# rubenwiersma/deltaconv

Measured on AMD Instinct MI355X. Metric: point-clouds/sec fwd+bwd, ModelNet40 1024pt k=20, 1/2/4/8 MI355X, higher is better.
Workload: dtype f32; 1 GPU; ModelNet40 classification, 1024 points, k=20, batch=32 per GPU, fwd+bwd+SGD step, train-mode BN/Dropout, HIP-graph replay; global_batch=32, parallelism=dp1

## Files before the change

deltaconv_amd/csrc/common.h:

```cpp
#pragma once
#include <hip/hip_runtime.h>
#include <stdint.h>
#include <stdio.h>

#define DC_EXPORT extern "C" __attribute__((visibility("default")))

enum {
    DC_OK = 0,
    DC_ERR_ARG = -1,
    DC_ERR_LAUNCH = -2,
    DC_ERR_WORKSPACE = -3
};

void dc_set_error(const char* fmt, ...);

#define DC_REQUIRE(cond, ...)                 \
    do {                                      \
        if (!(cond)) {                        \
            dc_set_error(__VA_ARGS__);        \
            return DC_ERR_ARG;                \
        }                                     \
    } while (0)

bool dc_ensure_lds(unsigned long long* done_mask, const void* kernel, size_t bytes, const char* what);
bool dc_take_lds_failure();

#define DC_CHECK_LAUNCH(name)                                                   \
    do {                                                                        \
        if (dc_take_lds_failure()) {                                            \
            (void)hipGetLastError();                                            \
            return DC_ERR_LAUNCH;                                               \
        }                                                                       \
        hipError_t e_ = hipGetLastError();                                      \
        if (e_ != hipSuccess) {                                                 \
            dc_set_error("%s: %s", name, hipGetErrorString(e_));                \
            return DC_ERR_LAUNCH;                                               \
        }                                                                       \
    } while (0)

enum { DC_OPT_XCD_REMAP = 0, DC_OPT_GATHER_BATCH = 1, DC_OPT_TN_LDS = 2 , DC_OPT_GEMM_EXACT = 3 , DC_OPT_GEMM_STAGGER = 4 , DC_OPT_TN_TILE = 5 , DC_OPT_TN_SLABS = 6 , DC_OPT_TILE_UPW = 7, DC_OPT_CSC_ONE_WG = 8 , DC_OPT_NO_PLANES = 9 , DC_OPT_CE_TWO_LAUNCH = 10 , DC_OPT_WIDE_TILES = 11 , DC_OPT_COUNT = 12 };
int dc_option(int key);

static inline int dc_cdiv(long long a, long long b) { return (int)((a + b - 1) / b); }

enum { DC_ST_TILE = 1 , DC_ST_ELL = 2 ,
       DC_ST_NN = 4 , DC_ST_GEMM = 8  };
#ifndef DC_NT_MASK
#define DC_NT_MASK (DC_ST_TILE)
#endif
typedef float dc_f32x4 __attribute__((ext_vector_type(4)));
template <int FAMILY>
__device__ __forceinline__ void dc_store16(float* p, dc_f32x4 v) {
    if constexpr ((DC_NT_MASK & FAMILY) != 0) __builtin_nontemporal_store(v, reinterpret_cast<dc_f32x4*>(p));
    else *reinterpret_cast<dc_f32x4*>(p) = v;
}

constexpr int DC_FIN_MAX = 4, DC_FIN_BLOB = 128;
enum { DC_FIN_BN = 0, DC_FIN_BWD_COEF = 1 };
struct DcFinPending {
    int kind, chunks, C;
    const double* partial;
    alignas(8) unsigned char blob[DC_FIN_BLOB];
    int stage1, rpc;
    long R;
    alignas(8) unsigned char functor[DC_FIN_BLOB];
};
bool dc_gemm_take_request();
void dc_gemm_flush(void* stream);
void dc_gemm_discard();
bool dc_fin_take_request();
void dc_fin_push(int kind, const double* partial, int chunks, int C, const void* fin, size_t bytes, const void* functor = nullptr,
                 size_t functor_bytes = 0, long R = 0, int rpc = 0);
int dc_fin_pending(DcFinPending** out);
// ... 46 lines not shown
```

deltaconv_amd/csrc/error.hip:

```cpp
#include <cstring>
#include "common.h"
#include <stdarg.h>

static thread_local char g_err[512] = "";

void dc_set_error(const char* fmt, ...) {
    va_list ap;
    va_start(ap, fmt);
    vsnprintf(g_err, sizeof(g_err), fmt, ap);
    va_end(ap);
}

DC_EXPORT const char* dc_last_error(void) { return g_err; }
DC_EXPORT int32_t dc_version(void) { return 100; }

static int g_opt[DC_OPT_COUNT] = {1};
int dc_option(int key) { return (key >= 0 && key < DC_OPT_COUNT) ? g_opt[key] : 0; }
DC_EXPORT int dc_set_option(int32_t key, int32_t value) {
    if (key < 0 || key >= DC_OPT_COUNT) return DC_ERR_ARG;
    g_opt[key] = value;
    return DC_OK;
}

static thread_local bool g_lds_failed = false;
bool dc_take_lds_failure() {
    const bool f = g_lds_failed;
    g_lds_failed = false;
    return f;
}
bool dc_ensure_lds(unsigned long long* done_mask, const void* kernel, size_t bytes, const char* what) {
    int dev = 0;
    if (hipGetDevice(&dev) != hipSuccess) dev = 0;
    const unsigned long long bit = dev < 64 ? 1ull << dev : 0ull;
    if (bit && (__atomic_load_n(done_mask, __ATOMIC_ACQUIRE) & bit)) return true;
    const hipError_t e = hipFuncSetAttribute(kernel, hipFuncAttributeMaxDynamicSharedMemorySize, (int)bytes);
    if (e != hipSuccess) {
        (void)hipGetLastError();
        dc_set_error("%s: needs %zu KiB of LDS per workgroup (MI355X / gfx950 offers 160 KiB); device %d refused: %s", what,
                     bytes / 1024, dev, hipGetErrorString(e));
        g_lds_failed = true;
        return false;
    }
    if (bit) __atomic_fetch_or(done_mask, bit, __ATOMIC_RELEASE);
    return true;
}

static thread_local DcFinPending g_fin[DC_FIN_MAX];
static thread_local int g_fin_count = 0;
static thread_local bool g_fin_open = false, g_fin_request = false, g_gemm_request = false;
bool dc_gemm_take_request() {
    const bool take = g_fin_open && g_gemm_request && g_fin_request;
    g_gemm_request = false;
    return take;
}
bool dc_fin_take_request() {
    const bool take = g_fin_open && g_fin_request && g_fin_count < DC_FIN_MAX;
    g_fin_request = false;
    return take;
}
void dc_fin_push(int kind, const double* partial, int chunks, int C, const void* fin, size_t bytes, const void* functor,
                 size_t functor_bytes, long R, int rpc) {
    DcFinPending& e = g_fin[g_fin_count++];
    e.kind = kind; e.partial = partial; e.chunks = chunks; e.C = C;
    memcpy(e.blob, fin, bytes);
    e.stage1 = functor != nullptr; e.R = R; e.rpc = rpc;
    if (functor) memcpy(e.functor, functor, functor_bytes);
}
int dc_fin_pending(DcFinPending** out) { *out = g_fin; return g_fin_count; }
void dc_fin_clear() { g_fin_count = 0; g_fin_open = false; g_fin_request = false; g_gemm_request = false; }
DC_EXPORT int dc_finalisers_begin(void) {
    if (g_fin_open) {
        dc_set_error("dc_finalisers_begin: a batch is already open on this thread");
        return DC_ERR_ARG;
    }
    g_fin_open = true; g_fin_count = 0; g_fin_request = false;
    return DC_OK;
}
DC_EXPORT int dc_finaliser_defer_next(void) {
    g_fin_request = g_fin_open;
    return DC_OK;
}
DC_EXPORT int dc_gemm_defer_next(void) {
    g_gemm_request = g_fin_open;
    return DC_OK;
// ... 23 lines not shown
```

deltaconv_amd/csrc/gemm.hip:

```cpp
#include <algorithm>
#include <type_traits>
#include "common.h"
#include "nn_math.h"
#include "colreduce.h"

namespace {

typedef float f32x16 __attribute__((ext_vector_type(16)));
typedef float f32x4 __attribute__((ext_vector_type(4)));

#ifndef DC_X3_PLAIN
#define DC_X3_PLAIN 2
#endif
#ifndef DC_X3_PRO
#define DC_X3_PRO 1
#endif
#ifdef DC_LAB_STAMPS
__device__ unsigned long long dc_lab_stamps[8192 * 8];
#define DC_STAMP(n) do { if (threadIdx.x == 0 && blockIdx.y == 0 && blockIdx.x < 8192) dc_lab_stamps[blockIdx.x * 8 + (n)] = __builtin_amdgcn_s_memtime(); } while (0)
#else
#define DC_STAMP(n) do { } while (0)
#endif
constexpr int BK = 32;
constexpr int LDK = BK + 4;
constexpr int NT = 256;

enum { EPI_NONE = 0, EPI_COLSTATS = 1, EPI_VNSTATS = 2 , EPI_VNSTATS0 = 3  };
enum { B_NK = 0 , B_KN = 1  };
enum { A_MK = 0 , A_KM = 1  };

struct GemmP {
    const float* A; long lda;
    const float* B; long ldb;
    float* C; long ldc;
    long M; int N; long K;
    int tiles_n, remap, accumulate;
    long k_per_slab, slab_stride;
    const float* A2; long lda2;
    const float* pc; int pcn;
    float slope;
    double* part; int chunks, stat_cols;
    int stagger, resident;
    const unsigned short* Bp; long bps;
};

typedef unsigned u32x4 __attribute__((ext_vector_type(4)));
__device__ __forceinline__ f32x4 uload4(const float* ubase, unsigned voff, unsigned soff = 0) {
    const __amdgpu_buffer_rsrc_t r = __builtin_amdgcn_make_buffer_rsrc(const_cast<float*>(ubase), 0, 0x7FFFFFFF, 0x00020000);
    const u32x4 v = __builtin_amdgcn_raw_buffer_load_b128(r, (int)voff, (int)soff, 0);
    return __builtin_bit_cast(f32x4, v);
}

constexpr unsigned POISON = 0x80000000u;
__device__ __forceinline__ f32x4 gload4v(const float* ubase, unsigned voff, unsigned soff, bool ok) {
    return uload4(ubase, ok ? voff : POISON, soff);
}
__device__ __forceinline__ f32x4 gload4s(const float* ubase, unsigned voff, unsigned soff, bool ok_row, long col, long ncols) {
    const __amdgpu_buffer_rsrc_t r = __builtin_amdgcn_make_buffer_rsrc(const_cast<float*>(ubase), 0, 0x7FFFFFFF, 0x00020000);
    f32x4 v;
#pragma unroll
    for (int e = 0; e < 4; ++e)
        v[e] = __builtin_bit_cast(float, __builtin_amdgcn_raw_buffer_load_b32(
                   r, (int)((ok_row && col + e < ncols) ? voff + 4u * e : POISON), (int)soff, 0));
    return v;
}
template <int MODE>
__device__ __forceinline__ f32x4 pload4(const float* ubase, unsigned voff, unsigned soff, bool ok_row, long col, long ncols) {
    if (MODE == 0) return uload4(ubase, voff, soff);
    if (MODE == 1) return gload4v(ubase, voff, soff, ok_row && col < ncols);
    return gload4s(ubase, voff, soff, ok_row, col, ncols);
}

__device__ __forceinline__ f32x4 bn_bwd_vec(const f32x4 dy, const f32x4 h, const f32x4 (&cf)[5], float slope) {
    f32x4 o;
#pragma unroll
    for (int e = 0; e < 4; ++e) {
        const float z = fmaf(cf[0][e], h[e], cf[1][e]);
        const float dz = dy[e] * (z > 0.f ? 1.f : slope);
        o[e] = fmaf(cf[2][e], dz, fmaf(cf[3][e], h[e], cf[4][e]));
// ... 2 lines not shown
}

__device__ __forceinline__ void lds_barrier() {
    __builtin_amdgcn_sched_barrier(0);
    asm volatile("s_waitcnt lgkmcnt(0)\n\ts_barrier" ::: "memory");
    __builtin_amdgcn_sched_barrier(0);
}

typedef __bf16 bf16x8 __attribute__((ext_vector_type(8)));
typedef __bf16 bf16x2 __attribute__((ext_vector_type(2)));
typedef float f32x2 __attribute__((ext_vector_type(2)));
struct Planes { u32x4 h, m, l; };
__device__ __forceinline__ unsigned pk_bf16(float a, float b) {
    return __builtin_bit_cast(unsigned, __builtin_convertvector((f32x2){a, b}, bf16x2));
}
__device__ __forceinline__ void split_pair(float x0, float x1, unsigned& h, unsigned& m, unsigned& l) {
    h = pk_bf16(x0, x1);
    const float r0 = x0 - __builtin_bit_cast(float, h << 16), r1 = x1 - __builtin_bit_cast(float, h & 0xFFFF0000u);
    m = pk_bf16(r0, r1);
    const float s0 = r0 - __builtin_bit_cast(float, m << 16), s1 = r1 - __builtin_bit_cast(float, m & 0xFFFF0000u);
    l = pk_bf16(s0, s1);
}
__device__ __forceinline__ void split8(const f32x4 a, const f32x4 b, Planes& o) {
    const float x[8] = {a[0], a[1], a[2], a[3], b[0], b[1], b[2], b[3]};
#pragma unroll
    for (int j = 0; j < 4; ++j) {
        unsigned h, m, l;
        split_pair(x[2 * j], x[2 * j + 1], h, m, l);
        o.h[j] = h; o.m[j] = m; o.l[j] = l;
    }
}
__device__ __forceinline__ f32x16 mfma_bf16(const u32x4 a, const u32x4 b, const f32x16 c) {
    return __builtin_amdgcn_mfma_f32_32x32x16_bf16(__builtin_bit_cast(bf16x8, a), __builtin_bit_cast(bf16x8, b), c, 0, 0, 0);
}

template <int BM, int BN, int AL, int BL, int MODE, int EPI, int PRO = 0, int X3 = 0, int BP = 0>
__device__ __forceinline__ void gemm_body(const GemmP& p, const unsigned bid, const unsigned gemm_blocks) {
    static_assert(!BP || (X3 == 2 && AL == A_MK && BL == B_NK && MODE == 0), "pre-split B planes: pipelined split loop, K-contiguous operands, whole tiles");
    constexpr bool FAST = MODE == 0;
    constexpr int MA = MODE == 0 ? 0 : (MODE == 1 || MODE == 3 ? 1 : 2), MB = MODE == 0 ? 0 : (MODE == 1 || MODE == 4 ? 1 : 2);
    constexpr int WM = BM / 2, WN = BN / 2;
    constexpr int TM = WM / 32, TN = WN / 32;
    constexpr int A_FL = AL == A_MK ? BM * LDK : BK * BM;
    constexpr int B_FL = BL == B_NK ? BN * LDK : BK * BN;
    constexpr int A_IT = BM / 32, B_IT = BP ? 0 : BN / 32;
    extern __shared__ __attribute__((aligned(16))) float smem[];
    float* As = smem;
    float* Bs = smem + 2 * A_FL;

    const int tid = threadIdx.x, lane = tid & 63, wave = tid >> 6;
    const int li = lane & 31, lh = lane >> 5;
    DC_STAMP(0);
    if (p.stagger > 0 && (long)blockIdx.y * gemm_blocks + bid < p.resident) {
        const unsigned slot = __builtin_amdgcn_s_getreg((3 << 11) | 4);
        if (slot & 1) {
            const unsigned long long t0 = __builtin_amdgcn_s_memtime();
            while (__builtin_amdgcn_s_memtime() - t0 < (unsigned long long)p.stagger) __builtin_amdgcn_s_sleep(16);
        }
    }
    long blk = bid;
    if (p.remap) {
        const long q = gemm_blocks >> 3, r = gemm_blocks & 7, xcd = blk & 7, idx = blk >> 3;
        blk = xcd * q + (xcd < r ? xcd : r) + idx;
    }
    const long kbeg = (long)blockIdx.y * p.k_per_slab;
    const long kend = min(p.K, kbeg + p.k_per_slab);
    const long tm = blk / p.tiles_n;
    const int tn = (int)(blk - tm * p.tiles_n);
    const long m0 = tm * BM;
    const int n0 = tn * BN;
    const int wm0 = (wave >> 1) * WM, wn0 = (wave & 1) * WN;

    f32x16 acc[TM][TN];
#pragma unroll
    for (int i = 0; i < TM; ++i)
#pragma unroll
        for (int j = 0; j < TN; ++j)
#pragma unroll
            for (int q = 0; q < 16; ++q) acc[i][j][q] = 0.f;

    constexpr int STG = (X3 || PRO || (BM == 128 && BN == 128 && BL == B_KN)) ? 1 : 2;
    f32x4 sa[STG][A_IT], sb[STG][B_IT ? B_IT : 1];
    f32x4 sa2[PRO ? A_IT : 1], cf[5];
    if (PRO && AL == A_KM) {
#pragma unroll
        for (int q = 0; q < 5; ++q)
            cf[q] = pload4<MODE == 0 ? 0 : 2>(p.pc + (long)q * p.pcn + m0, (unsigned)((tid % (BM / 4)) * 16), 0, true,
                                              m0 + (tid % (BM / 4)) * 4, p.M);
    }
    const unsigned voa = AL == A_MK ? (unsigned)(((tid >> 3) * p.lda + (tid & 7) * 4) * 4)
                                    : (unsigned)(((tid / (BM / 4)) * p.lda + (tid % (BM / 4)) * 4) * 4);
    const unsigned voa2 = AL == A_MK ? (unsigned)(((tid >> 3) * p.lda2 + (tid & 7) * 4) * 4)
// ... 483 lines not shown
                        float yu, yv;
                        dcnn::vn_combine(pu, qu, pv, qv, yu, yv);
                        const double nr = (double)dcnn::vn_norm(yu, yv);
                        s0 += nr;
                        s1 += nr * nr;
                    }
                }
            }
            s0 += __shfl_xor(s0, 32, 64);
            s1 += __shfl_xor(s1, 32, 64);
            if (lh == 0) {
                if (EPI == EPI_COLSTATS || EPI == EPI_VNSTATS0) {
                    const int c = wn0 + jn * 32 + li;
                    sst[(0 * 2 + (wave >> 1)) * SC + c] = s0;
                    sst[(1 * 2 + (wave >> 1)) * SC + c] = s1;
                } else if ((li & 1) == 0) {
                    const int c = (wn0 + jn * 32 + li) >> 1;
                    sst[(0 * 2 + (wave >> 1)) * SC + c] = s0;
                    sst[(1 * 2 + (wave >> 1)) * SC + c] = s1;
                }
            }
        }
        __syncthreads();
        for (int idx = tid; idx < 2 * SC; idx += NT) {
            const int q = idx / SC, c = idx - q * SC;
            const int gc = (EPI == EPI_VNSTATS ? n0 / 2 : n0) + c;
            if (gc < p.stat_cols)
                p.part[((long)q * p.stat_cols + gc) * p.chunks + tm] = sst[(q * 2 + 0) * SC + c] + sst[(q * 2 + 1) * SC + c];
        }
        __syncthreads();
    }

    DC_STAMP(3);
    float* stg = smem + wave * (WM * WN);
#pragma unroll
    for (int i = 0; i < TM; ++i)
#pragma unroll
        for (int jn = 0; jn < TN; ++jn)
#pragma unroll
            for (int q = 0; q < 16; ++q)
                stg[(i * 32 + (q & 3) + 8 * (q >> 2) + 4 * lh) * WN + jn * 32 + li] = acc[i][jn][q];
    __syncthreads();
    float* cbase = p.C + (long)blockIdx.y * p.slab_stride;
    constexpr int RL = WN / 4;
#pragma unroll
    for (int it = 0; it < WM * WN / 4 / 64; ++it) {
        const int idx = it * 64 + lane;
        const int r = idx / RL, c4 = (idx % RL) * 4;
        const long row = m0 + wm0 + r;
        const int col = n0 + wn0 + c4;
        f32x4 v = *reinterpret_cast<const f32x4*>(stg + r * WN + c4);
        float* dst = cbase + row * p.ldc + col;
        if (FAST) {
            if (p.accumulate) {
                const f32x4 o = *reinterpret_cast<const f32x4*>(dst);
                v += o;
            }
            dc_store16<DC_ST_GEMM>(dst, v);
        } else if (row < p.M) {
            if (col + 3 < p.N && (reinterpret_cast<uintptr_t>(dst) & 15) == 0) {
                if (p.accumulate) {
                    const f32x4 o = *reinterpret_cast<const f32x4*>(dst);
                    v += o;
                }
                dc_store16<DC_ST_GEMM>(dst, v);
            } else {
#pragma unroll
                for (int e = 0; e < 4; ++e)
                    if (col + e < p.N) dst[e] = p.accumulate ? dst[e] + v[e] : v[e];
            }
        }
    }
    DC_STAMP(4);
#ifdef DC_LAB_STAMPS
    asm volatile("s_waitcnt vmcnt(0)" ::: "memory");
    DC_STAMP(5);
    if (threadIdx.x == 0 && blockIdx.y == 0 && blockIdx.x < 8192) dc_lab_stamps[blockIdx.x * 8 + 6] = __builtin_amdgcn_s_getreg((16 << 11) | 4);
#endif
}

template <int BM, int BN, int AL, int BL, int MODE, int EPI, int PRO = 0, int X3 = 0, int BP = 0>
__global__ __launch_bounds__(NT, 2) void gemm_kernel(GemmP p) {
    gemm_body<BM, BN, AL, BL, MODE, EPI, PRO, X3, BP>(p, blockIdx.x, gridDim.x);
}
template <int BM, int BN, int AL, int BL, int MODE, int EPI, int PRO = 0, int X3 = 0, int BP = 0>
__global__ __launch_bounds__(NT, 2) void gemm_pair_kernel(GemmP p0, GemmP p1, unsigned nb0) {
    if (blockIdx.x < nb0) gemm_body<BM, BN, AL, BL, MODE, EPI, PRO, X3, BP>(p0, blockIdx.x, nb0);
    else gemm_body<BM, BN, AL, BL, MODE, EPI, PRO, X3, BP>(p1, blockIdx.x - nb0, gridDim.x - nb0);
}

struct Tile { int bm, bn; };

Tile pick_tile(long M, int N, int K, int tile) {
    switch (tile) {
        case 1: return {128, 128};
        case 2: return {128, 64};
        case 3: return {64, 64};
        case 4: return {64, 128};
        default: break;
    }
    int bn = N > 64 ? 128 : 64;
    if (N % 128 != 0 && N % 64 == 0) bn = 64;
    long tn = (N + bn - 1) / bn;
    int bm = ((M + 127) / 128) * tn >= 384 ? 128 : 64;
    if (M % bm != 0 && M % 64 == 0) bm = 64;
    if (bm == 64 && bn == 128 && N % 64 == 0 && ((M + 63) / 64) * tn < 256 && dc_option(DC_OPT_WIDE_TILES) == 0) bn = 64;
    return {bm, bn};
}

size_t lds_bytes(int bm, int bn, int al, int bl) {
    const size_t a = al == A_MK ? (size_t)bm * LDK : (size_t)BK * bm, b = bl == B_NK ? (size_t)bn * LDK : (size_t)BK * bn;
    return std::max(2 * (a + b), (size_t)bm * bn) * sizeof(float);
}

typedef void (*GemmSingleFn)(const GemmP&, unsigned, size_t, hipStream_t);
typedef void (*GemmPairFn)(const GemmP&, const GemmP&, unsigned, unsigned, size_t, hipStream_t);
struct GemmPending { GemmP p; unsigned blocks; size_t lds; GemmSingleFn single; GemmPairFn pair; };
static thread_local GemmPending g_gemm_q[DC_FIN_MAX];
static thread_local int g_gemm_n = 0;

template <int BM, int BN, int AL, int BL, int MODE, int EPI, int PRO, int X3, int BP>
void gemm_single_thunk(const GemmP& p, unsigned blocks, size_t lds, hipStream_t s) {
    hipLaunchKernelGGL((gemm_kernel<BM, BN, AL, BL, MODE, EPI, PRO, X3, BP>), dim3(blocks, 1), dim3(NT), lds, s, p);
}
template <int BM, int BN, int AL, int BL, int MODE, int EPI, int PRO, int X3, int BP>
void gemm_pair_thunk(const GemmP& p0, const GemmP& p1, unsigned b0, unsigned b1, size_t lds, hipStream_t s) {
    static unsigned long long configured = 0;
    if (!dc_ensure_lds(&configured, reinterpret_cast<const void*>(&gemm_pair_kernel<BM, BN, AL, BL, MODE, EPI, PRO, X3, BP>), lds, "dense product pair"))
        return;
    GemmP q1 = p1;
    q1.stagger = 0;
    hipLaunchKernelGGL((gemm_pair_kernel<BM, BN, AL, BL, MODE, EPI, PRO, X3, BP>), dim3(b0 + b1, 1), dim3(NT), lds, s, p0, q1, b0);
}

template <int BM, int BN, int AL, int BL, int MODE, int EPI, int PRO, int X3, int BP = 0>
void launch_one(const GemmP& p, long tiles_m, int slabs, hipStream_t s) {
    static unsigned long long configured = 0;
    const size_t lds = lds_bytes(BM, BN, AL, BL);
    if (!dc_ensure_lds(&configured, reinterpret_cast<const void*>(&gemm_kernel<BM, BN, AL, BL, MODE, EPI, PRO, X3, BP>), lds, "dense product")) return;
    constexpr bool PAIRABLE = EPI == EPI_COLSTATS && BP == 1 && MODE == 0 && PRO == 0 && AL == A_MK && BL == B_NK;
    if (dc_gemm_take_request()) {
        if constexpr (PAIRABLE) {
            if (slabs == 1 && g_gemm_n < DC_FIN_MAX) {
                GemmPending& e = g_gemm_q[g_gemm_n++];
                e.p = p; e.blocks = (unsigned)(tiles_m * p.tiles_n); e.lds = lds;
                e.single = &gemm_single_thunk<BM, BN, AL, BL, MODE, EPI, PRO, X3, BP>;
                e.pair = &gemm_pair_thunk<BM, BN, AL, BL, MODE, EPI, PRO, X3, BP>;
                return;
            }
        }
    }
    hipLaunchKernelGGL((gemm_kernel<BM, BN, AL, BL, MODE, EPI, PRO, X3, BP>),
                       dim3((unsigned)(tiles_m * p.tiles_n), (unsigned)slabs), dim3(NT), lds, s, p);
}

template <int AL, int BL, int MODE, int EPI, int PRO, int X3 = 0, int BP = 0>
void launch_tile(const GemmP& p, Tile t, long tiles_m, int slabs, hipStream_t s) {
    if (t.bm == 128 && t.bn == 128) launch_one<128, 128, AL, BL, MODE, EPI, PRO, X3, BP>(p, tiles_m, slabs, s);
    else if (t.bm == 128) launch_one<128, 64, AL, BL, MODE, EPI, PRO, X3, BP>(p, tiles_m, slabs, s);
    else if (t.bn == 128) launch_one<64, 128, AL, BL, MODE, EPI, PRO, X3, BP>(p, tiles_m, slabs, s);
    else launch_one<64, 64, AL, BL, MODE, EPI, PRO, X3, BP>(p, tiles_m, slabs, s);
}

template <int AL, int BL, int EPI, int PRO = 0>
void launch_fast(const GemmP& p, Tile t, long tiles_m, int slabs, int mode, hipStream_t s) {
    const bool split = mode == 0 && (dc_option(DC_OPT_GEMM_EXACT) == 2 ||
                                     (dc_option(DC_OPT_GEMM_EXACT) == 0 && t.bn == 128 && (AL == A_MK || t.bm == 128)));
    if constexpr (AL == A_MK && BL == B_NK) {
        if (p.Bp && mode == 0 && dc_option(DC_OPT_GEMM_EXACT) == 0) {
            launch_tile<AL, BL, 0, EPI, PRO, 2, 1>(p, t, tiles_m, slabs, s);
            return;
        }
    }
    if (split) launch_tile<AL, BL, 0, EPI, PRO, (PRO ? DC_X3_PRO : DC_X3_PLAIN)>(p, t, tiles_m, slabs, s);
    else if (mode == 0) launch_tile<AL, BL, 0, EPI, PRO>(p, t, tiles_m, slabs, s);
    else if (mode == 1) launch_tile<AL, BL, 1, EPI, PRO>(p, t, tiles_m, slabs, s);
    else if (mode == 2) launch_tile<AL, BL, 2, EPI, PRO>(p, t, tiles_m, slabs, s);
    else if (mode == 3) launch_tile<AL, BL, 3, EPI, PRO>(p, t, tiles_m, slabs, s);
    else launch_tile<AL, BL, 4, EPI, PRO>(p, t, tiles_m, slabs, s);
}

int load_mode(bool whole_tiles, bool a4, bool b4) {
    if (whole_tiles && a4 && b4) return 0;
    return a4 && b4 ? 1 : (a4 ? 3 : (b4 ? 4 : 2));
}

void set_stagger(GemmP& p, Tile t, long workgroups, long k_per_wg) {
    p.stagger = 0;
    p.resident = 512;
    int pct = dc_option(DC_OPT_GEMM_STAGGER);
    if (pct == 0) pct = 50;
    if (pct < 0 || t.bm != 128 || t.bn != 128 || workgroups < 2 * p.resident) return;
    const long per_tile = dc_option(DC_OPT_GEMM_EXACT) ? 4200 : 1250;
    p.stagger = (int)std::min<long>((k_per_wg + BK - 1) / BK * per_tile * pct / 100, 400000);
}

bool al16p(const void* q) { return (reinterpret_cast<uintptr_t>(q) & 15) == 0; }

struct Prologue { const float* h; long ldh; const float* coefs; int ncoef; float slope; };
struct BHint { const void* src; const unsigned short* p; long stride, ld; int transposed; };
thread_local BHint g_bhint = {nullptr, nullptr, 0, 0, 0};

int run_gemm(const char* name, int bl, int epi, const float* A, long lda, const float* B, long ldb, long M, int N, int K,
// ... 334 lines not shown
```

Measured before the change: 11330 clouds/s.

## Add specialised 128-wide split-bf16 GEMM kernel with register-streamed B planes

```diff
diff --git a/deltaconv_amd/csrc/common.h b/deltaconv_amd/csrc/common.h
--- a/deltaconv_amd/csrc/common.h
+++ b/deltaconv_amd/csrc/common.h
@@ -38,7 +38,7 @@
         }                                                                       \
     } while (0)
 
-enum { DC_OPT_XCD_REMAP = 0, DC_OPT_GATHER_BATCH = 1, DC_OPT_TN_LDS = 2 , DC_OPT_GEMM_EXACT = 3 , DC_OPT_GEMM_STAGGER = 4 , DC_OPT_TN_TILE = 5 , DC_OPT_TN_SLABS = 6 , DC_OPT_TILE_UPW = 7, DC_OPT_CSC_ONE_WG = 8 , DC_OPT_NO_PLANES = 9 , DC_OPT_CE_TWO_LAUNCH = 10 , DC_OPT_WIDE_TILES = 11 , DC_OPT_COUNT = 12 };
+enum { DC_OPT_XCD_REMAP = 0, DC_OPT_GATHER_BATCH = 1, DC_OPT_TN_LDS = 2 , DC_OPT_GEMM_EXACT = 3 , DC_OPT_GEMM_STAGGER = 4 , DC_OPT_TN_TILE = 5 , DC_OPT_TN_SLABS = 6 , DC_OPT_TILE_UPW = 7, DC_OPT_CSC_ONE_WG = 8 , DC_OPT_NO_PLANES = 9 , DC_OPT_CE_TWO_LAUNCH = 10 , DC_OPT_WIDE_TILES = 11 , DC_OPT_GEMM_TILE128 = 12 , DC_OPT_COUNT = 13 };
 int dc_option(int key);
 
 static inline int dc_cdiv(long long a, long long b) { return (int)((a + b - 1) / b); }
diff --git a/deltaconv_amd/csrc/error.hip b/deltaconv_amd/csrc/error.hip
--- a/deltaconv_amd/csrc/error.hip
+++ b/deltaconv_amd/csrc/error.hip
@@ -49,7 +49,7 @@
 static thread_local int g_fin_count = 0;
 static thread_local bool g_fin_open = false, g_fin_request = false, g_gemm_request = false;
 bool dc_gemm_take_request() {
-    const bool take = g_fin_open && g_gemm_request && g_fin_request;
+    const bool take = g_fin_open && g_gemm_request && g_fin_request && g_fin_count < DC_FIN_MAX;
     g_gemm_request = false;
     return take;
 }
diff --git a/deltaconv_amd/csrc/gemm.hip b/deltaconv_amd/csrc/gemm.hip
--- a/deltaconv_amd/csrc/gemm.hip
+++ b/deltaconv_amd/csrc/gemm.hip
@@ -745,6 +745,229 @@
     else gemm_body<BM, BN, AL, BL, MODE, EPI, PRO, X3, BP>(p1, blockIdx.x - nb0, gridDim.x - nb0);
 }
 
+constexpr int PLK = BK + 8;
+template <int BM, int EPI>
+__device__ __forceinline__ void gemm_sas_body(const GemmP& p, const unsigned bid, const unsigned gemm_blocks) {
+    constexpr int BN = 128, NTW = 2 * BM, TM = 2, TN = 2, WM = 64, WN = 64, NWR = BM / 64;
+    constexpr int A_IT = BM * BK / 4 / NTW;
+    constexpr int PL = BM * PLK;
+    extern __shared__ __attribute__((aligned(16))) float smem[];
+    unsigned short* const Ap = reinterpret_cast<unsigned short*>(smem);
+
+    const int tid = threadIdx.x, lane = tid & 63, wave = tid >> 6;
+    const int li = lane & 31, lh = lane >> 5;
+    DC_STAMP(0);
+    long blk = bid;
+    if (p.remap) {
+        const long q = gemm_blocks >> 3, r = gemm_blocks & 7, xcd = blk & 7, idx = blk >> 3;
+        blk = xcd * q + (xcd < r ? xcd : r) + idx;
+    }
+    const long tm = blk / p.tiles_n;
+    const int tn = (int)(blk - tm * p.tiles_n);
+    const long m0 = tm * BM;
+    const int n0 = tn * BN;
+    const int wm0 = (wave >> 1) * WM, wn0 = (wave & 1) * WN;
+
+    f32x16 acc[TM][TN];
+#pragma unroll
+    for (int i = 0; i < TM; ++i)
+#pragma unroll
+        for (int j = 0; j < TN; ++j)
+#pragma unroll
+            for (int q = 0; q < 16; ++q) acc[i][j][q] = 0.f;
+
+    const float* const ua = p.A + m0 * p.lda;
+    const unsigned voa = (unsigned)(((tid >> 3) * p.lda + (tid & 7) * 4) * 4);
+    f32x4 sa[A_IT];
+    auto gload = [&](int it, long k0) {
+        sa[it] = uload4(ua + k0, voa, (unsigned)(it * (NTW / 8) * 4) * (unsigned)p.lda);
+    };
+    auto sstore = [&](int it, int buf) {
+        unsigned h0, m0_, l0, h1, m1, l1;
+        split_pair(sa[it][0], sa[it][1], h0, m0_, l0);
+        split_pair(sa[it][2], sa[it][3], h1, m1, l1);
+        unsigned short* d = Ap + buf * 3 * PL + ((tid >> 3) + it * (NTW / 8)) * PLK + (tid & 7) * 4;
+        *reinterpret_cast<uint2*>(d) = make_uint2(h0, h1);
+        *reinterpret_cast<uint2*>(d + PL) = make_uint2(m0_, m1);
+        *reinterpret_cast<uint2*>(d + 2 * PL) = make_uint2(l0, l1);
+    };
+    auto aread = [&](Planes (&o)[TM], int buf, int ks) {
+#pragma unroll
+        for (int i = 0; i < TM; ++i) {
+            const unsigned short* a = Ap + buf * 3 * PL + (wm0 + 32 * i + li) * PLK + 16 * ks + 8 * lh;
+            o[i].h = *reinterpret_cast<const u32x4*>(a);
+            o[i].m = *reinterpret_cast<const u32x4*>(a + PL);
+            o[i].l = *reinterpret_cast<const u32x4*>(a + 2 * PL);
+        }
+    };
+    const __amdgpu_buffer_rsrc_t rbp = __builtin_amdgcn_make_buffer_rsrc(const_cast<unsigned short*>(p.Bp), 0, 0x7FFFFFFF, 0x00020000);
+    const unsigned vobp = (unsigned)(lane * 16);
+    const unsigned ksteps = (unsigned)(p.ldb >> 4);
+    auto bload = [&](Planes (&o)[TN], long k) {
+#pragma unroll
+        for (int jn = 0; jn < TN; ++jn) {
+            const unsigned so = (((unsigned)((n0 + wn0) >> 5) + (unsigned)jn) * ksteps + (unsigned)(k >> 4)) * 1024u;
+            o[jn].h = __builtin_amdgcn_raw_buffer_load_b128(rbp, (int)vobp, (int)so, 0);
+            o[jn].m = __builtin_amdgcn_raw_buffer_load_b128(rbp, (int)vobp, (int)(so + (unsigned)(p.bps * 2)), 0);
+            o[jn].l = __builtin_amdgcn_raw_buffer_load_b128(rbp, (int)vobp, (int)(so + (unsigned)(p.bps * 4)), 0);
+        }
+    };
+    auto mma = [&](const Planes (&a)[TM], const Planes (&b)[TN]) {
+#pragma unroll
+        for (int pr = 0; pr < 6; ++pr)
+#pragma unroll
+            for (int i = 0; i < TM; ++i)
+#pragma unroll
+                for (int jn = 0; jn < TN; ++jn) {
+                    const u32x4 x = pr == 0 ? a[i].l : (pr == 2 || pr == 3 ? a[i].m : a[i].h);
+                    const u32x4 y = pr == 1 ? b[jn].l : (pr == 2 || pr == 4 ? b[jn].m : b[jn].h);
+                    acc[i][jn] = mfma_bf16(x, y, acc[i][jn]);
+                }
+    };
+
+    DC_STAMP(1);
+    const int nk = (int)(p.K / BK);
+    Planes pa[2][TM], pb[2][TN];
+#pragma unroll
+    for (int it = 0; it < A_IT; ++it) gload(it, 0);
+#pragma unroll
+    for (int it = 0; it < A_IT; ++it) sstore(it, 0);
+    if (nk > 1) {
+#pragma unroll
+        for (int it = 0; it < A_IT; ++it) gload(it, BK);
+    }
+    bload(pb[0], 0);
+    bload(pb[1], 16);
+    lds_barrier();
+    DC_STAMP(7);
+    aread(pa[0], 0, 0);
+    for (int kt = 0; kt < nk; ++kt) {
+        const int cur = kt & 1;
+        const bool more = kt + 1 < nk, more2 = kt + 2 < nk;
+        const long kn = (long)(kt + 1) * BK;
+        aread(pa[1], cur, 1);
+        mma(pa[0], pb[0]);
+        if (more) {
+            bload(pb[0], kn);
+#pragma unroll
+            for (int it = 0; it < A_IT / 2; ++it) sstore(it, cur ^ 1);
+        }
+        if (more2) {
+#pragma unroll
+            for (int it = 0; it < A_IT / 2; ++it) gload(it, kn + BK);
+        }
+        mma(pa[1], pb[1]);
+        if (more) {
+            bload(pb[1], kn + 16);
+#pragma unroll
+            for (int it = A_IT / 2; it < A_IT; ++it) sstore(it, cur ^ 1);
+        }
+        if (more2) {
+#pragma unroll
+            for (int it = A_IT / 2; it < A_IT; ++it) gload(it, kn + BK);
+        }
+        lds_barrier();
+        if (more) aread(pa[0], cur ^ 1, 0);
+    }
+    DC_STAMP(2);
+    __syncthreads();
+
+    if (EPI != EPI_NONE) {
+        constexpr int SC = EPI == EPI_VNSTATS ? BN / 2 : BN;
+        double* sst = reinterpret_cast<double*>(smem);
+#pragma unroll
+        for (int jn = 0; jn < TN; ++jn) {
+            double s0 = 0.0, s1 = 0.0;
+#pragma unroll
+            for (int i = 0; i < TM; ++i) {
+                if (EPI == EPI_COLSTATS) {
+#pragma unroll
+                    for (int q = 0; q < 16; ++q) {
+                        const double x = (double)acc[i][jn][q];
+                        s0 += x;
+                        s1 += x * x;
+                    }
+                } else if (EPI == EPI_VNSTATS0) {
+#pragma unroll
+                    for (int q = 0; q < 16; q += 2) {
+                        const double nr = (double)dcnn::vn_norm(acc[i][jn][q], acc[i][jn][q + 1]);
+                        s0 += nr;
+                        s1 += nr * nr;
+                    }
+                } else {
+#pragma unroll
+                    for (int q = 0; q < 16; q += 2) {
+                        const float pu = acc[i][jn][q], pv = acc[i][jn][q + 1];
+                        const float qu = __shfl_xor(pu, 1, 64), qv = __shfl_xor(pv, 1, 64);
+                        float yu, yv;
+                        dcnn::vn_combine(pu, qu, pv, qv, yu, yv);
+                        const double nr = (double)dcnn::vn_norm(yu, yv);
+                        s0 += nr;
+                        s1 += nr * nr;
+                    }
+                }
+            }
+            s0 += __shfl_xor(s0, 32, 64);
+            s1 += __shfl_xor(s1, 32, 64);
+            if (lh == 0) {
+                if (EPI == EPI_COLSTATS || EPI == EPI_VNSTATS0) {
+                    const int c = wn0 + jn * 32 + li;
+                    sst[(0 * NWR + (wave >> 1)) * SC + c] = s0;
+                    sst[(1 * NWR + (wave >> 1)) * SC + c] = s1;
+                } else if ((li & 1) == 0) {
+                    const int c = (wn0 + jn * 32 + li) >> 1;
+                    sst[(0 * NWR + (wave >> 1)) * SC + c] = s0;
+                    sst[(1 * NWR + (wave >> 1)) * SC + c] = s1;
+                }
+            }
+        }
+        __syncthreads();
+        for (int idx = tid; idx < 2 * SC * (NWR / 2); idx += NTW) {
+            const int ch = idx / (2 * SC), rem = idx - ch * 2 * SC, q = rem / SC, c = rem - q * SC;
+            const int gc = (EPI == EPI_VNSTATS ? n0 / 2 : n0) + c;
+            if (gc < p.stat_cols)
+                p.part[((long)q * p.stat_cols + gc) * p.chunks + tm * (NWR / 2) + ch] =
+                    sst[(q * NWR + 2 * ch) * SC + c] + sst[(q * NWR + 2 * ch + 1) * SC + c];
+        }
+        __syncthreads();
+    }
+
+    DC_STAMP(3);
+    float* stg = smem + wave * (WM * WN);
+#pragma unroll
+    for (int i = 0; i < TM; ++i)
+#pragma unroll
+        for (int jn = 0; jn < TN; ++jn)
+#pragma unroll
+            for (int q = 0; q < 16; ++q)
+                stg[(i * 32 + (q & 3) + 8 * (q >> 2) + 4 * lh) * WN + jn * 32 + li] = acc[i][jn][q];
+    __syncthreads();
+    constexpr int RL = WN / 4;
+#pragma unroll
+    for (int it = 0; it < WM * WN / 4 / 64; ++it) {
+        const int idx = it * 64 + lane;
+        const int r = idx / RL, c4 = (idx % RL) * 4;
+        f32x4 v = *reinterpret_cast<const f32x4*>(stg + r * WN + c4);
+        float* dst = p.C + (m0 + wm0 + r) * p.ldc + n0 + wn0 + c4;
+        if (p.accumulate) {
+            const f32x4 o = *reinterpret_cast<const f32x4*>(dst);
+            v += o;
+        }
+        dc_store16<DC_ST_GEMM>(dst, v);
+    }
+    DC_STAMP(4);
+}
+
+template <int BM, int EPI>
+__global__ __launch_bounds__(2 * BM, BM == 128 ? 2 : 1) void gemm_sas_kernel(GemmP p) {
+    gemm_sas_body<BM, EPI>(p, blockIdx.x, gridDim.x);
+}
+template <int BM, int EPI>
+__global__ __launch_bounds__(2 * BM, BM == 128 ? 2 : 1) void gemm_sas_pair_kernel(GemmP p0, GemmP p1, unsigned nb0) {
+    if (blockIdx.x < nb0) gemm_sas_body<BM, EPI>(p0, blockIdx.x, nb0);
+    else gemm_sas_body<BM, EPI>(p1, blockIdx.x - nb0, gridDim.x - nb0);
+}
+
 struct Tile { int bm, bn; };
 
 Tile pick_tile(long M, int N, int K, int tile) {
@@ -782,8 +1005,12 @@
 template <int BM, int BN, int AL, int BL, int MODE, int EPI, int PRO, int X3, int BP>
 void gemm_pair_thunk(const GemmP& p0, const GemmP& p1, unsigned b0, unsigned b1, size_t lds, hipStream_t s) {
     static unsigned long long configured = 0;
-    if (!dc_ensure_lds(&configured, reinterpret_cast<const void*>(&gemm_pair_kernel<BM, BN, AL, BL, MODE, EPI, PRO, X3, BP>), lds, "dense product pair"))
+    if (!dc_ensure_lds(&configured, reinterpret_cast<const void*>(&gemm_pair_kernel<BM, BN, AL, BL, MODE, EPI, PRO, X3, BP>), lds, "dense product pair")) {
+        (void)dc_take_lds_failure();
+        gemm_single_thunk<BM, BN, AL, BL, MODE, EPI, PRO, X3, BP>(p0, b0, lds, s);
+        gemm_single_thunk<BM, BN, AL, BL, MODE, EPI, PRO, X3, BP>(p1, b1, lds, s);
         return;
+    }
     GemmP q1 = p1;
     q1.stagger = 0;
     hipLaunchKernelGGL((gemm_pair_kernel<BM, BN, AL, BL, MODE, EPI, PRO, X3, BP>), dim3(b0 + b1, 1), dim3(NT), lds, s, p0, q1, b0);
@@ -818,12 +1045,64 @@
     else launch_one<64, 64, AL, BL, MODE, EPI, PRO, X3, BP>(p, tiles_m, slabs, s);
 }
 
+int sas_rows(const GemmP& p, Tile t) {
+    const int opt = dc_option(DC_OPT_GEMM_TILE128);
+    if (opt == 1 || t.bm != 128 || t.bn != 128 || p.N % 128 != 0 || p.M % 128 != 0 || p.K % BK != 0) return 0;
+    if (opt == 3) return p.M % 256 == 0 ? 256 : 0;
+    return 128;
+}
+size_t sas_lds_bytes(int bm) {
+    return std::max((size_t)2 * 3 * bm * PLK * sizeof(unsigned short), (size_t)bm * 128 * sizeof(float));
+}
+template <int BM, int EPI>
+void sas_single_thunk(const GemmP& p, unsigned blocks, size_t lds, hipStream_t s) {
+    hipLaunchKernelGGL((gemm_sas_kernel<BM, EPI>), dim3(blocks), dim3(2 * BM), lds, s, p);
+}
+template <int BM, int EPI>
+void sas_pair_thunk(const GemmP& p0, const GemmP& p1, unsigned b0, unsigned b1, size_t lds, hipStream_t s) {
+    static unsigned long long configured = 0;
+    if (!dc_ensure_lds(&configured, reinterpret_cast<const void*>(&gemm_sas_pair_kernel<BM, EPI>), lds, "dense product pair")) {
+        (void)dc_take_lds_failure();
+        sas_single_thunk<BM, EPI>(p0, b0, lds, s);
+        sas_single_thunk<BM, EPI>(p1, b1, lds, s);
+        return;
+    }
+    hipLaunchKernelGGL((gemm_sas_pair_kernel<BM, EPI>), dim3(b0 + b1), dim3(2 * BM), lds, s, p0, p1, b0);
+}
+template <int BM, int EPI>
+void launch_sas_one(const GemmP& p, hipStream_t s) {
+    static unsigned long long configured = 0;
+    const size_t lds = sas_lds_bytes(BM);
+    if (!dc_ensure_lds(&configured, reinterpret_cast<const void*>(&gemm_sas_kernel<BM, EPI>), lds, "dense product")) return;
+    const unsigned blocks = (unsigned)((p.M / BM) * p.tiles_n);
+    if (dc_gemm_take_request()) {
+        if (EPI == EPI_COLSTATS && g_gemm_n < DC_FIN_MAX) {
+            GemmPending& e = g_gemm_q[g_gemm_n++];
+            e.p = p; e.blocks = blocks; e.lds = lds;
+            e.single = &sas_single_thunk<BM, EPI>;
+            e.pair = &sas_pair_thunk<BM, EPI>;
+            return;
+        }
+    }
+    sas_single_thunk<BM, EPI>(p, blocks, lds, s);
+}
+template <int EPI>
+bool launch_sas(const GemmP& p, Tile t, hipStream_t s) {
+    const int bm = sas_rows(p, t);
+    if (bm == 256) launch_sas_one<256, EPI>(p, s);
+    else if (bm == 128) launch_sas_one<128, EPI>(p, s);
+    return bm != 0;
+}
+
 template <int AL, int BL, int EPI, int PRO = 0>
 void launch_fast(const GemmP& p, Tile t, long tiles_m, int slabs, int mode, hipStream_t s) {
     const bool split = mode == 0 && (dc_option(DC_OPT_GEMM_EXACT) == 2 ||
                                      (dc_option(DC_OPT_GEMM_EXACT) == 0 && t.bn == 128 && (AL == A_MK || t.bm == 128)));
     if constexpr (AL == A_MK && BL == B_NK) {
         if (p.Bp && mode == 0 && dc_option(DC_OPT_GEMM_EXACT) == 0) {
+            if constexpr (PRO == 0) {
+                if (slabs == 1 && launch_sas<EPI>(p, t, s)) return;
+            }
             launch_tile<AL, BL, 0, EPI, PRO, 2, 1>(p, t, tiles_m, slabs, s);
             return;
         }
```

New measurement: 11340 clouds/s (median of 6 runs). About the same (+0.1%).

## Add transposed-LDS image kernel for weight-gradient GEMM with bf16x3 split

Applied to the files above, without the earlier changes.

```diff
diff --git a/deltaconv_amd/csrc/common.h b/deltaconv_amd/csrc/common.h
--- a/deltaconv_amd/csrc/common.h
+++ b/deltaconv_amd/csrc/common.h
@@ -38,7 +38,7 @@
         }                                                                       \
     } while (0)
 
-enum { DC_OPT_XCD_REMAP = 0, DC_OPT_GATHER_BATCH = 1, DC_OPT_TN_LDS = 2 , DC_OPT_GEMM_EXACT = 3 , DC_OPT_GEMM_STAGGER = 4 , DC_OPT_TN_TILE = 5 , DC_OPT_TN_SLABS = 6 , DC_OPT_TILE_UPW = 7, DC_OPT_CSC_ONE_WG = 8 , DC_OPT_NO_PLANES = 9 , DC_OPT_CE_TWO_LAUNCH = 10 , DC_OPT_WIDE_TILES = 11 , DC_OPT_COUNT = 12 };
+enum { DC_OPT_XCD_REMAP = 0, DC_OPT_GATHER_BATCH = 1, DC_OPT_TN_LDS = 2 , DC_OPT_GEMM_EXACT = 3 , DC_OPT_GEMM_STAGGER = 4 , DC_OPT_TN_TILE = 5 , DC_OPT_TN_SLABS = 6 , DC_OPT_TILE_UPW = 7, DC_OPT_CSC_ONE_WG = 8 , DC_OPT_NO_PLANES = 9 , DC_OPT_CE_TWO_LAUNCH = 10 , DC_OPT_WIDE_TILES = 11 , DC_OPT_WGRAD_IMAGE = 12 , DC_OPT_COUNT = 13 };
 int dc_option(int key);
 
 static inline int dc_cdiv(long long a, long long b) { return (int)((a + b - 1) / b); }
diff --git a/deltaconv_amd/csrc/gemm.hip b/deltaconv_amd/csrc/gemm.hip
--- a/deltaconv_amd/csrc/gemm.hip
+++ b/deltaconv_amd/csrc/gemm.hip
@@ -3,6 +3,7 @@
 #include "common.h"
 #include "nn_math.h"
 #include "colreduce.h"
+#include "wgrad_image_layout.h"
 
 namespace {
 
@@ -45,6 +46,7 @@
 };
 
 typedef unsigned u32x4 __attribute__((ext_vector_type(4)));
+typedef unsigned u32x2 __attribute__((ext_vector_type(2)));
 __device__ __forceinline__ f32x4 uload4(const float* ubase, unsigned voff, unsigned soff = 0) {
     const __amdgpu_buffer_rsrc_t r = __builtin_amdgcn_make_buffer_rsrc(const_cast<float*>(ubase), 0, 0x7FFFFFFF, 0x00020000);
     const u32x4 v = __builtin_amdgcn_raw_buffer_load_b128(r, (int)voff, (int)soff, 0);
@@ -113,6 +115,61 @@
 }
 __device__ __forceinline__ f32x16 mfma_bf16(const u32x4 a, const u32x4 b, const f32x16 c) {
     return __builtin_amdgcn_mfma_f32_32x32x16_bf16(__builtin_bit_cast(bf16x8, a), __builtin_bit_cast(bf16x8, b), c, 0, 0, 0);
+}
+
+template <int BM, int BN, bool FAST>
+__device__ __forceinline__ void store_tile(const GemmP& p, const f32x16 (&acc)[BM / 64][BN / 64], float* smem, long row0, int col0) {
+    constexpr int WM = BM / 2, WN = BN / 2, TM = WM / 32, TN = WN / 32;
+    const int lane = threadIdx.x & 63, wave = threadIdx.x >> 6, li = lane & 31, lh = lane >> 5;
+    float* stg = smem + wave * (WM * WN);
+#pragma unroll
+    for (int i = 0; i < TM; ++i)
+#pragma unroll
+        for (int jn = 0; jn < TN; ++jn)
+#pragma unroll
+            for (int q = 0; q < 16; ++q)
+                stg[(i * 32 + (q & 3) + 8 * (q >> 2) + 4 * lh) * WN + jn * 32 + li] = acc[i][jn][q];
+    __syncthreads();
+    float* cbase = p.C + (long)blockIdx.y * p.slab_stride;
+    constexpr int RL = WN / 4;
+#pragma unroll
+    for (int it = 0; it < WM * WN / 4 / 64; ++it) {
+        const int idx = it * 64 + lane;
+        const int r = idx / RL, c4 = (idx % RL) * 4;
+        const long row = row0 + r;
+        const int col = col0 + c4;
+        f32x4 v = *reinterpret_cast<const f32x4*>(stg + r * WN + c4);
+        float* dst = cbase + row * p.ldc + col;
+        if (FAST) {
+            if (p.accumulate) {
+                const f32x4 o = *reinterpret_cast<const f32x4*>(dst);
+                v += o;
+            }
+            dc_store16<DC_ST_GEMM>(dst, v);
+        } else if (row < p.M) {
+            if (col + 3 < p.N && (reinterpret_cast<uintptr_t>(dst) & 15) == 0) {
+                if (p.accumulate) {
+                    const f32x4 o = *reinterpret_cast<const f32x4*>(dst);
+                    v += o;
+                }
+                dc_store16<DC_ST_GEMM>(dst, v);
+            } else {
+#pragma unroll
+                for (int e = 0; e < 4; ++e)
+                    if (col + e < p.N) dst[e] = p.accumulate ? dst[e] + v[e] : v[e];
+            }
+        }
+    }
+}
+
+__device__ __forceinline__ void stagger_wait(const GemmP& p, const unsigned bid, const unsigned gemm_blocks) {
+    if (p.stagger > 0 && (long)blockIdx.y * gemm_blocks + bid < p.resident) {
+        const unsigned slot = __builtin_amdgcn_s_getreg((3 << 11) | 4);
+        if (slot & 1) {
+            const unsigned long long t0 = __builtin_amdgcn_s_memtime();
+            while (__builtin_amdgcn_s_memtime() - t0 < (unsigned long long)p.stagger) __builtin_amdgcn_s_sleep(16);
+        }
+    }
 }
 
 template <int BM, int BN, int AL, int BL, int MODE, int EPI, int PRO = 0, int X3 = 0, int BP = 0>
@@ -132,13 +189,7 @@
     const int tid = threadIdx.x, lane = tid & 63, wave = tid >> 6;
     const int li = lane & 31, lh = lane >> 5;
     DC_STAMP(0);
-    if (p.stagger > 0 && (long)blockIdx.y * gemm_blocks + bid < p.resident) {
-        const unsigned slot = __builtin_amdgcn_s_getreg((3 << 11) | 4);
-        if (slot & 1) {
-            const unsigned long long t0 = __builtin_amdgcn_s_memtime();
-            while (__builtin_amdgcn_s_memtime() - t0 < (unsigned long long)p.stagger) __builtin_amdgcn_s_sleep(16);
-        }
-    }
+    stagger_wait(p, bid, gemm_blocks);
     long blk = bid;
     if (p.remap) {
         const long q = gemm_blocks >> 3, r = gemm_blocks & 7, xcd = blk & 7, idx = blk >> 3;
@@ -688,45 +739,7 @@
     }
 
     DC_STAMP(3);
-    float* stg = smem + wave * (WM * WN);
-#pragma unroll
-    for (int i = 0; i < TM; ++i)
-#pragma unroll
-        for (int jn = 0; jn < TN; ++jn)
-#pragma unroll
-            for (int q = 0; q < 16; ++q)
-                stg[(i * 32 + (q & 3) + 8 * (q >> 2) + 4 * lh) * WN + jn * 32 + li] = acc[i][jn][q];
-    __syncthreads();
-    float* cbase = p.C + (long)blockIdx.y * p.slab_stride;
-    constexpr int RL = WN / 4;
-#pragma unroll
-    for (int it = 0; it < WM * WN / 4 / 64; ++it) {
-        const int idx = it * 64 + lane;
-        const int r = idx / RL, c4 = (idx % RL) * 4;
-        const long row = m0 + wm0 + r;
-        const int col = n0 + wn0 + c4;
-        f32x4 v = *reinterpret_cast<const f32x4*>(stg + r * WN + c4);
-        float* dst = cbase + row * p.ldc + col;
-        if (FAST) {
-            if (p.accumulate) {
-                const f32x4 o = *reinterpret_cast<const f32x4*>(dst);
-                v += o;
-            }
-            dc_store16<DC_ST_GEMM>(dst, v);
-        } else if (row < p.M) {
-            if (col + 3 < p.N && (reinterpret_cast<uintptr_t>(dst) & 15) == 0) {
-                if (p.accumulate) {
-                    const f32x4 o = *reinterpret_cast<const f32x4*>(dst);
-                    v += o;
-                }
-                dc_store16<DC_ST_GEMM>(dst, v);
-            } else {
-#pragma unroll
-                for (int e = 0; e < 4; ++e)
-                    if (col + e < p.N) dst[e] = p.accumulate ? dst[e] + v[e] : v[e];
-            }
-        }
-    }
+    store_tile<BM, BN, FAST>(p, acc, smem, m0 + wm0, n0 + wn0);
     DC_STAMP(4);
 #ifdef DC_LAB_STAMPS
     asm volatile("s_waitcnt vmcnt(0)" ::: "memory");
@@ -744,6 +757,8 @@
     if (blockIdx.x < nb0) gemm_body<BM, BN, AL, BL, MODE, EPI, PRO, X3, BP>(p0, blockIdx.x, nb0);
     else gemm_body<BM, BN, AL, BL, MODE, EPI, PRO, X3, BP>(p1, blockIdx.x - nb0, gridDim.x - nb0);
 }
+
+#include "wgrad_image.h"
 
 struct Tile { int bm, bn; };
 
@@ -818,6 +833,16 @@
     else launch_one<64, 64, AL, BL, MODE, EPI, PRO, X3, BP>(p, tiles_m, slabs, s);
 }
 
+template <int PRO>
+void launch_wgi(const GemmP& p, Tile t, long tiles_m, int slabs, hipStream_t s) {
+    const size_t ring = 2 * 3 * (size_t)dcwg::KS * (t.bm + t.bn) * 2, lds = std::max(ring, (size_t)t.bm * t.bn * sizeof(float));
+    const dim3 grid((unsigned)(tiles_m * p.tiles_n), (unsigned)slabs);
+    if (t.bm == 128 && t.bn == 128) hipLaunchKernelGGL((gemm_wgi_kernel<128, 128, PRO>), grid, dim3(NT), lds, s, p);
+    else if (t.bm == 128) hipLaunchKernelGGL((gemm_wgi_kernel<128, 64, PRO>), grid, dim3(NT), lds, s, p);
+    else if (t.bn == 128) hipLaunchKernelGGL((gemm_wgi_kernel<64, 128, PRO>), grid, dim3(NT), lds, s, p);
+    else hipLaunchKernelGGL((gemm_wgi_kernel<64, 64, PRO>), grid, dim3(NT), lds, s, p);
+}
+
 template <int AL, int BL, int EPI, int PRO = 0>
 void launch_fast(const GemmP& p, Tile t, long tiles_m, int slabs, int mode, hipStream_t s) {
     const bool split = mode == 0 && (dc_option(DC_OPT_GEMM_EXACT) == 2 ||
@@ -825,6 +850,13 @@
     if constexpr (AL == A_MK && BL == B_NK) {
         if (p.Bp && mode == 0 && dc_option(DC_OPT_GEMM_EXACT) == 0) {
             launch_tile<AL, BL, 0, EPI, PRO, 2, 1>(p, t, tiles_m, slabs, s);
+            return;
+        }
+    }
+    if constexpr (AL == A_KM && BL == B_KN) {
+        const int img = dc_option(DC_OPT_WGRAD_IMAGE);
+        if (mode == 0 && img != 1 && dc_option(DC_OPT_GEMM_EXACT) != 1 && (split || img == 3)) {
+            launch_wgi<PRO>(p, t, tiles_m, slabs, s);
             return;
         }
     }
diff --git a/deltaconv_amd/csrc/wgrad_image.h b/deltaconv_amd/csrc/wgrad_image.h
--- /dev/null
+++ b/deltaconv_amd/csrc/wgrad_image.h
@@ -0,0 +1,156 @@
+template <int BM, int BN, int PRO>
+__device__ __forceinline__ void wgrad_image_body(const GemmP& p) {
+    using dcwg::KS;
+    constexpr int WM = BM / 2, WN = BN / 2, TM = WM / 32, TN = WN / 32;
+    constexpr int A_PL = KS * BM * 2, B_PL = KS * BN * 2;
+    constexpr int STAGE = 3 * (A_PL + B_PL);
+    constexpr int A_IT = KS * BM / 4 / NT, B_IT = KS * BN / 4 / NT;
+    constexpr int NP = A_IT + B_IT;
+    constexpr int STG = PRO ? 1 : 2;
+    constexpr int NM = 6 * TM * TN, NF = TM + TN, NR = 6 * NF;
+    constexpr int CR = (NR + NM - 1) / NM;
+    static_assert(NT == dcwg::WG && A_IT >= 1 && B_IT >= 1, "tile / workgroup shape");
+    extern __shared__ __attribute__((aligned(16))) float smem[];
+    unsigned char* const lds = reinterpret_cast<unsigned char*>(smem);
+
+    const int tid = threadIdx.x, lane = tid & 63, wave = tid >> 6;
+    stagger_wait(p, blockIdx.x, gridDim.x);
+    const long kbeg = (long)blockIdx.y * p.k_per_slab;
+    const long kend = min(p.K, kbeg + p.k_per_slab);
+    const long tm = blockIdx.x / p.tiles_n;
+    const int tn = (int)(blockIdx.x - tm * p.tiles_n);
+    const long m0 = tm * BM;
+    const int n0 = tn * BN;
+    const int wm0 = (wave >> 1) * WM, wn0 = (wave & 1) * WN;
+    const int ns = (int)((kend - kbeg) / KS);
+
+    f32x16 acc[TM][TN];
+#pragma unroll
+    for (int i = 0; i < TM; ++i)
+#pragma unroll
+        for (int j = 0; j < TN; ++j)
+#pragma unroll
+            for (int q = 0; q < 16; ++q) acc[i][j][q] = 0.f;
+
+    f32x4 sa[STG][A_IT], sb[STG][B_IT], sa2[STG][PRO ? A_IT : 1], cf[5];
+    const int ca = dcwg::piece_col(BM, tid, 0), cb = dcwg::piece_col(BN, tid, 0);
+    if (PRO) {
+#pragma unroll
+        for (int q = 0; q < 5; ++q) cf[q] = uload4(p.pc + (long)q * p.pcn + m0, (unsigned)(ca * 4));
+    }
+    const unsigned voa = (unsigned)((dcwg::piece_row(BM, tid, 0) * p.lda + ca) * 4);
+    const unsigned voa2 = (unsigned)((dcwg::piece_row(BM, tid, 0) * p.lda2 + ca) * 4);
+    const unsigned vob = (unsigned)((dcwg::piece_row(BN, tid, 0) * p.ldb + cb) * 4);
+    auto load_piece = [&](int n, int t, auto set_tag) {
+        constexpr int S = decltype(set_tag)::value;
+        const long k0 = kbeg + (long)min(t, ns - 1) * KS;
+        if (n < A_IT) {
+            const unsigned rows = (unsigned)(n * (NT / (BM / 4)));
+            sa[S][n] = uload4(p.A + k0 * p.lda + m0, voa, rows * 4u * (unsigned)p.lda);
+            if (PRO) sa2[S][n] = uload4(p.A2 + k0 * p.lda2 + m0, voa2, rows * 4u * (unsigned)p.lda2);
+        } else {
+            const int it = n - A_IT;
+            const unsigned rows = (unsigned)(it * (NT / (BN / 4)));
+            sb[S][it] = uload4(p.B + k0 * p.ldb + n0, vob, rows * 4u * (unsigned)p.ldb);
+        }
+    };
+    auto store_piece = [&](int n, int buf, auto set_tag) {
+        constexpr int S = decltype(set_tag)::value;
+        const bool isa = n < A_IT;
+        const int it = isa ? n : n - A_IT, width = isa ? BM : BN, plane = isa ? A_PL : B_PL;
+        const f32x4 v = isa ? (PRO ? bn_bwd_vec(sa[S][it], sa2[S][it], cf, p.slope) : sa[S][it]) : sb[S][it];
+        unsigned h0, m0_, l0, h1, m1, l1;
+        split_pair(v[0], v[1], h0, m0_, l0);
+        split_pair(v[2], v[3], h1, m1, l1);
+        unsigned char* d = lds + buf * STAGE + (isa ? 0 : 3 * A_PL) +
+                           dcwg::img_off(width, dcwg::piece_row(width, tid, it), isa ? ca : cb);
+        *reinterpret_cast<uint2*>(d) = make_uint2(h0, h1);
+        *reinterpret_cast<uint2*>(d + plane) = make_uint2(m0_, m1);
+        *reinterpret_cast<uint2*>(d + 2 * plane) = make_uint2(l0, l1);
+    };
+    unsigned tra[TM][2], trb[TN][2];
+#pragma unroll
+    for (int i = 0; i < TM; ++i)
+#pragma unroll
+        for (int h = 0; h < 2; ++h) tra[i][h] = dcwg::tr_off(BM, wm0 + 32 * i, lane, h);
+#pragma unroll
+    for (int jn = 0; jn < TN; ++jn)
+#pragma unroll
+        for (int h = 0; h < 2; ++h) trb[jn][h] = dcwg::tr_off(BN, wn0 + 32 * jn, lane, h);
+    typedef short v4i16 __attribute__((ext_vector_type(4)));
+    typedef __attribute__((address_space(3))) v4i16 lds_v4i16;
+    auto tr_read = [&](unsigned byte_off) -> u32x2 {
+        return __builtin_bit_cast(u32x2, __builtin_amdgcn_ds_read_tr16_b64_v4i16((lds_v4i16*)(lds + byte_off)));
+    };
+    auto read_one = [&](int r, int buf, Planes (&pa)[TM], Planes (&pb)[TN]) {
+        const int f = r / 6, pl = (r % 6) / 2, h = r % 2;
+        const bool isa = f < TM;
+        const unsigned o = buf * STAGE + (isa ? pl * A_PL + tra[f][h] : 3 * A_PL + pl * B_PL + trb[f - TM][h]);
+        const u32x2 v = tr_read(o);
+        Planes& d = isa ? pa[f] : pb[f - TM];
+        u32x4& w = pl == 0 ? d.h : (pl == 1 ? d.m : d.l);
+        w[2 * h] = v[0];
+        w[2 * h + 1] = v[1];
+    };
+    auto mfma_one = [&](int g, const Planes (&ca_)[TM], const Planes (&cb_)[TN]) {
+        const int pr = g / (TM * TN), r = g % (TM * TN), i = r / TN, jn = r % TN;
+        const u32x4 a = pr == 0 ? ca_[i].l : (pr == 2 || pr == 3 ? ca_[i].m : ca_[i].h);
+        const u32x4 b = pr == 1 ? cb_[jn].l : (pr == 2 || pr == 4 ? cb_[jn].m : cb_[jn].h);
+        acc[i][jn] = mfma_bf16(a, b, acc[i][jn]);
+    };
+
+    Planes pa0[TM], pb0[TN], pa1[TM], pb1[TN];
+    using S0 = std::integral_constant<int, 0>;
+    using S1 = std::integral_constant<int, STG - 1>;
+#pragma unroll
+    for (int n = 0; n < NP; ++n) load_piece(n, 0, S0{});
+#pragma unroll
+    for (int n = 0; n < NP; ++n) store_piece(n, 0, S0{});
+#pragma unroll
+    for (int n = 0; n < NP; ++n) load_piece(n, 1, S1{});
+#pragma unroll
+    for (int n = 0; n < NP; ++n) store_piece(n, 1, S1{});
+#pragma unroll
+    for (int n = 0; n < NP; ++n) load_piece(n, 2, S0{});
+    if (STG == 2) {
+#pragma unroll
+        for (int n = 0; n < NP; ++n) load_piece(n, 3, S1{});
+    }
+    lds_barrier();
+#pragma unroll
+    for (int r = 0; r < NR; ++r) read_one(r, 0, pa0, pb0);
+
+    auto stage = [&](int s, auto par_tag, const Planes (&ca_)[TM], const Planes (&cb_)[TN], Planes (&na)[TM], Planes (&nb)[TN]) {
+        constexpr int PAR = decltype(par_tag)::value;
+        using SS = std::integral_constant<int, STG == 2 ? PAR : 0>;
+#pragma unroll
+        for (int g = 0; g < NM; ++g) {
+            mfma_one(g, ca_, cb_);
+#pragma unroll
+            for (int c = 0; c < CR; ++c)
+                if (g * CR + c < NR) read_one(g * CR + c, PAR ^ 1, na, nb);
+#pragma unroll
+            for (int n = 0; n < NP; ++n) {
+                if (n * NM / NP == g) {
+                    store_piece(n, PAR, SS{});
+                    load_piece(n, s + 2 + STG, SS{});
+                }
+            }
+            __builtin_amdgcn_sched_barrier(0);
+        }
+        lds_barrier();
+    };
+    using P0 = std::integral_constant<int, 0>;
+    using P1 = std::integral_constant<int, 1>;
+    for (int s = 0; s < ns; s += 2) {
+        stage(s, P0{}, pa0, pb0, pa1, pb1);
+        stage(s + 1, P1{}, pa1, pb1, pa0, pb0);
+    }
+    __syncthreads();
+    store_tile<BM, BN, true>(p, acc, smem, m0 + wm0, n0 + wn0);
+}
+
+template <int BM, int BN, int PRO>
+__global__ __launch_bounds__(NT, 2) void gemm_wgi_kernel(GemmP p) {
+    wgrad_image_body<BM, BN, PRO>(p);
+}
diff --git a/deltaconv_amd/csrc/wgrad_image_layout.h b/deltaconv_amd/csrc/wgrad_image_layout.h
--- /dev/null
+++ b/deltaconv_amd/csrc/wgrad_image_layout.h
@@ -0,0 +1,28 @@
+#pragma once
+
+#if defined(__HIPCC__)
+#define DCWG_HD __host__ __device__ __forceinline__
+#else
+#define DCWG_HD inline
+#endif
+
+namespace dcwg {
+
+constexpr int KS = 16;
+constexpr int WG = 256;
+
+DCWG_HD unsigned img_off(int width, int row, int col) {
+    const unsigned ch = (unsigned)col >> 3, half = ((unsigned)col >> 2) & 1u, r = (unsigned)row;
+    if (width == 128) return 256u * r + 16u * (ch ^ (((r & 3u) << 2) | ((r >> 2) & 3u))) + 8u * half;
+    return 128u * r + 16u * (ch ^ (((r >> 1) & 1u) << 2)) + 8u * half;
+}
+
+DCWG_HD unsigned tr_off(int width, int c0, int lane, int rd) {
+    const int g = lane >> 4, w = lane & 15;
+    return img_off(width, 8 * (g >> 1) + 4 * rd + (w >> 2), c0 + 16 * (g & 1) + 4 * (w & 3));
+}
+
+DCWG_HD int piece_row(int width, int tid, int it) { return (tid + WG * it) / (width / 4); }
+DCWG_HD int piece_col(int width, int tid, int it) { return ((tid + WG * it) % (width / 4)) * 4; }
+
+}
```

New measurement: 11000 clouds/s before, 11090 clouds/s after, median of 6. Within noise of the previous version (+0.8%).
